# zerohd4869/MM-DFN

Measured on AMD Instinct MI355X. Metric: utterances/sec (fwd+bwd), IEMOCAP-shaped batch, higher is better.
Workload: dtype f32; 1 GPU; cfg2 (BASELINE configs[1]): B=16 dialogues/GPU, L=110, dims 100/100/512, 2 GCN layers, P=2, dropout 0.50; utterances_per_gpu=1760, parallelism=dp1

## Files before the change

mm_dfn_amd/csrc/gcn_stack.hip:

```cpp
#include "mmdfn_internal.h"
#include "../../include/mmdfn_hip.h"
#include "stack_image_map.h"
#include <stdlib.h>

namespace {

constexpr int RB = 16;

__device__ __forceinline__ float4 zero4() { return make_float4(0.f, 0.f, 0.f, 0.f); }
__device__ __forceinline__ float4 one4() { return make_float4(1.f, 1.f, 1.f, 1.f); }
__device__ __forceinline__ float4 mul4(float4 a, float4 b) { return make_float4(a.x * b.x, a.y * b.y, a.z * b.z, a.w * b.w); }
__device__ __forceinline__ float4 scl4(float4 a, float s) { return make_float4(a.x * s, a.y * s, a.z * s, a.w * s); }
__device__ __forceinline__ float4 add4(float4 a, float4 b) { return make_float4(a.x + b.x, a.y + b.y, a.z + b.z, a.w + b.w); }
__device__ __forceinline__ float4 fma4(float4 a, float s, float4 b) { return make_float4(a.x * s + b.x, a.y * s + b.y, a.z * s + b.z, a.w * s + b.w); }

typedef float f32x2_t __attribute__((ext_vector_type(2)));
__device__ __forceinline__ void st4_nt(float* p, float4 v) { __builtin_nontemporal_store((f32x4){v.x, v.y, v.z, v.w}, reinterpret_cast<f32x4*>(p)); }
__device__ __forceinline__ void nt_store2(float* p, float2 v) { __builtin_nontemporal_store((f32x2_t){v.x, v.y}, reinterpret_cast<f32x2_t*>(p)); }
__device__ __forceinline__ int frag_row(int i) { return i < 4 ? 2 * i : (i < 12 ? 2 * (i - 4) + 1 : 2 * (i - 12) + 8); }
__device__ __forceinline__ int frag_unit(int g) { return ((g & 1) << 1) | (g >> 1); }

__host__ __device__ inline int lds_stride(int K) {
    int ld = ((K + 15) & ~15) + 4;
    if (((ld >> 2) & 1) == 0) ld += 4;
// ... 904 lines not shown
        const float gi = rgi[s_].F, gf = rgf[s_].F, gg = rgg[s_].F, go = rgo[s_].F; \
        const float tc = tanhf_(rcn[s_].F);                                         \
        const float dhv = rdh[s_].F + rdh2[s_].F;                                   \
        const float dc = rdc[s_].F + dhv * go * (1.0f - tc * tc);                   \
        dO.F = dhv * tc * go * (1.0f - go);                                         \
        di.F = dc * gg * gi * (1.0f - gi);                                          \
        df.F = dc * rcp[s_].F * gf * (1.0f - gf);                                   \
        dg.F = dc * gi * (1.0f - gg * gg);                                          \
        dcp.F = dc * gf;                                                            \
    }
            GB1(x) GB1(y) GB1(z) GB1(w)
#undef GB1
            float* sp = dst + r * ldw + u;
            st4(sp, di); st4(sp + H, df); st4(sp + 2 * H, dg); st4(sp + 3 * H, dO);
            if (writer && row < R) {
                float* d = dG + (int64_t)row * 4 * H + u;
                st4(d, di); st4(d + H, df); st4(d + 2 * H, dg); st4(d + 3 * H, dO);
                if (has_h) st4(dc_prev + (int64_t)row * H + u, dcp);
            }
        }
    };
    if ((int)blockIdx.x < nrb) issue(blockIdx.x);
    wst.commit(sW, ldw, ncols, K);
    if (ncols < CBW) {
        for (int i = threadIdx.x; i < (CBW - ncols) * (ldw >> 2); i += 256) st4(sW + ncols * ldw + 4 * i, zero4());
    }
    zero_pads(sA, 2 * RB, ldw, K);
    if ((int)blockIdx.x < nrb) park(blockIdx.x, sA);
    __syncthreads();
    const int er = threadIdx.x >> 4, en = (threadIdx.x & 15) * 4;
    int buf = 0;
    FOR_ROW_BLOCKS(rb, nrb) {
        const int nxt = rb + gridDim.x;
        if (nxt < nrb) issue(nxt);
        const int erow = rb * RB + er;
        const bool eok = en < ncols && erow < R;
        const float4 rv = (!is_dh && dres && eok) ? ld4(dres + (int64_t)erow * lddres + n0 + en) : zero4();
        f32x4 acc[1] = {{0.f, 0.f, 0.f, 0.f}};
        float* Acur = sA + buf * RB * ldw;
        contract<1>(acc, wrow0, Acur, ldw, sW, ldw, K);
        __syncthreads();
        spill_tiles<1>(acc, wrow0, nt, Acur, ldp);
        __syncthreads();
        if (eok) {
            const float4 v = add4(ld4(Acur + er * ldp + en), rv);
            st4((is_dh ? dh_prev : dq) + (int64_t)erow * H + n0 + en, v);
        }
        if (nxt < nrb) park(nxt, sA + (buf ^ 1) * RB * ldw);
        __syncthreads();
        buf ^= 1;
    }
}

template <int ABL, bool WIDE = false, bool IMG = false>
__global__ __launch_bounds__(512) void lstm_gate_bwd_ws_kernel(const float* __restrict__ gates, const float* __restrict__ c_prev,
                                                               const float* __restrict__ c_new, const float* __restrict__ dh_a,
                                                               const float* __restrict__ dh_b, const float* __restrict__ dc_next,
                                                               const float* __restrict__ Wih, const float* __restrict__ Whh,
                                                               const float* __restrict__ dres, float* __restrict__ dG,
                                                               float* __restrict__ dc_prev, float* __restrict__ dq,
                                                               float* __restrict__ dh_prev, int R, int H, int has_h,
                                                               int lddres, const float4* __restrict__ img) {
    static_assert(!(IMG && WIDE), "the image form keeps the two-column-block launch");
    extern __shared__ __attribute__((aligned(16))) float smem[];
    const int K = 4 * H;
    const int ldw = lds_stride(K);
    float* sW = smem;
    float* sA = IMG ? smem : sW + CBW * ldw;
    const int nb = WIDE ? 1 : (H + CBW - 1) / CBW;
    const bool is_dh = (int)blockIdx.y >= nb;
    const int n0 = WIDE ? 0 : (is_dh ? blockIdx.y - nb : blockIdx.y) * CBW;
    const int ncols = min(CBW, H - n0);
    const int nrb = (R + RB - 1) / RB;
    const int tid = threadIdx.x & 255;
    const bool producer = threadIdx.x >= 256;
    const int nyb = gridDim.y, yb = blockIdx.y;
    const bool wr_i = (0 % nyb) == yb, wr_f = (1 % nyb) == yb, wr_g = (2 % nyb) == yb, wr_o = (3 % nyb) == yb, wr_c = yb == nyb - 1;
    const int H4 = H >> 2;
    const float rH4 = 1.0f / (float)H4;
    ImageFrags<1, IMG ? GATE_BWD_NKM : 1> wim;
    if constexpr (IMG) {
        const int cw = tid >> 6;
        const int tile0[1] = {16 * cw < ncols ? 16 * cw : 0};
        if (!producer) wim.load(img, tile0, CBW / 16, blockIdx.y, (K + 15) >> 4);
        const int np4 = (ldw - K) >> 2;
        const float rnp4 = 1.0f / (float)(np4 > 0 ? np4 : 1);
        for (int i = threadIdx.x; i < 2 * RB * np4; i += 512) { const int r = qdiv(i, rnp4), j = i - r * np4; st4(sA + r * ldw + K + 4 * j, zero4()); }
    } else {
        const float* Wsrc = is_dh ? Whh : Wih;
        const int inner = ncols >> 2;
        const int total = K * inner;
        constexpr int NW2 = 13;
        float4 v[NW2];
#pragma unroll
        for (int e = 0; e < NW2; ++e) {
            const int i0 = threadIdx.x + 512 * e, i = i0 < total ? i0 : total - 1;
            const int r = i / inner, j = i - r * inner;
            v[e] = ld4(Wsrc + (int64_t)r * H + n0 + 4 * j);
        }
#pragma unroll
        for (int e = 0; e < NW2; ++e) {
            const int i = threadIdx.x + 512 * e;
            if (i >= total) continue;
            const int r = i / inner, j = i - r * inner;
            float* d = sW + (4 * j) * ldw + r;
            d[0] = v[e].x; d[ldw] = v[e].y; d[2 * ldw] = v[e].z; d[3 * ldw] = v[e].w;
        }
        const int np4 = (ldw - K) >> 2;
        const float rnp4 = 1.0f / (float)(np4 > 0 ? np4 : 1);
        for (int i = threadIdx.x; i < ncols * np4; i += 512) { const int r = qdiv(i, rnp4), j = i - r * np4; st4(sW + r * ldw + K + 4 * j, zero4()); }
        for (int i = threadIdx.x; i < (CBW - ncols) * (ldw >> 2); i += 512) st4(sW + ncols * ldw + 4 * i, zero4());
        for (int i = threadIdx.x; i < 2 * RB * np4; i += 512) { const int r = qdiv(i, rnp4), j = i - r * np4; st4(sA + r * ldw + K + 4 * j, zero4()); }
    }
    constexpr int NS = 2;
    float4 rgi[NS], rgf[NS], rgg[NS], rgo[NS], rcn[NS], rcp[NS], rdh[NS], rdh2[NS], rdc[NS];
    auto issue = [&](int rb) {
#pragma unroll
        for (int s_ = 0; s_ < NS; ++s_) {
            const int i = tid + 256 * s_;
            const int r = qdiv(i, rH4), u = (i - r * H4) * 4, row = rb * RB + r;
            const bool ok = !(ABL & 2) && i < RB * H4 && row < R;
            const int64_t o = (int64_t)row * H + u;
            const float* gr = gates + (int64_t)row * 4 * H + u;
            rgi[s_] = ok ? ld4(gr) : zero4();
            rgf[s_] = ok ? ld4(gr + H) : zero4();
            rgg[s_] = ok ? ld4(gr + 2 * H) : zero4();
            rgo[s_] = ok ? ld4(gr + 3 * H) : zero4();
            rcn[s_] = ok ? ld4(c_new + o) : zero4();
            rcp[s_] = (ok && c_prev) ? ld4(c_prev + o) : zero4();
            rdh[s_] = (ok && dh_a) ? ld4(dh_a + o) : zero4();
            rdh2[s_] = (ok && dh_b) ? ld4(dh_b + o) : zero4();
            rdc[s_] = (ok && dc_next) ? ld4(dc_next + o) : zero4();
        }
    };
    float4 odi[NS], odf[NS], odg[NS], odo[NS], odc[NS];
    auto park = [&](float* dst) {
#pragma unroll
        for (int s_ = 0; s_ < NS; ++s_) {
            const int i = tid + 256 * s_;
            float4 di, df, dg, dO, dcp;
#define GB1(F)                                                                      \
    {                                                                               \
        const float gi = rgi[s_].F, gf = rgf[s_].F, gg = rgg[s_].F, go = rgo[s_].F; \
        const float tc = tanhf_(rcn[s_].F);                                         \
        const float dhv = rdh[s_].F + rdh2[s_].F;                                   \
        const float dc = rdc[s_].F + dhv * go * (1.0f - tc * tc);                   \
        dO.F = dhv * tc * go * (1.0f - go);                                         \
        di.F = dc * gg * gi * (1.0f - gi);                                          \
        df.F = dc * rcp[s_].F * gf * (1.0f - gf);                                   \
        dg.F = dc * gi * (1.0f - gg * gg);                                          \
        dcp.F = dc * gf;                                                            \
    }
            if (ABL & 4) { di = rgi[s_]; df = rgf[s_]; dg = rgg[s_]; dO = rgo[s_]; dcp = rcn[s_]; }
            else { GB1(x) GB1(y) GB1(z) GB1(w) }
#undef GB1
            odi[s_] = di; odf[s_] = df; odg[s_] = dg; odo[s_] = dO; odc[s_] = dcp;
            if (i >= RB * H4) continue;
            const int r = qdiv(i, rH4), u = (i - r * H4) * 4;
            float* sp = dst + r * ldw + u;
            st4(sp, di); st4(sp + H, df); st4(sp + 2 * H, dg); st4(sp + 3 * H, dO);
        }
    };
    auto flush = [&](int rb) {
        if (ABL & 8) return;
#pragma unroll
        for (int s_ = 0; s_ < NS; ++s_) {
            const int i = tid + 256 * s_;
            if (i >= RB * H4) continue;
            const int r = qdiv(i, rH4), u = (i - r * H4) * 4, row = rb * RB + r;
            if (row >= R) continue;
            float* d = dG + (int64_t)row * 4 * H + u;
            if (wr_i) st4_nt(d, odi[s_]);
            if (wr_f) st4_nt(d + H, odf[s_]);
            if (wr_g) st4_nt(d + 2 * H, odg[s_]);
            if (wr_o) st4_nt(d + 3 * H, odo[s_]);
            if (has_h && wr_c) st4(dc_prev + (int64_t)row * H + u, odc[s_]);
        }
    };
    const int first = blockIdx.x, stride = gridDim.x;
    if (producer) {
        if (first < nrb) { issue(first); park(sA); }
        if (first + stride < nrb) issue(first + stride);
        if (first < nrb) flush(first);
    }
    __syncthreads();
    const int w = tid >> 6, lane = tid & 63, fi = lane & 15, g = lane >> 4;
    const int wrow0[1] = {16 * w < ncols ? 16 * w : 0};
    const int ecol = n0 + 16 * w + frag_row(fi);
    const bool ecol_ok = (16 * w + frag_row(fi)) < ncols;
    float* const outp = is_dh ? dh_prev : dq;
    constexpr int NKC = WIDE ? GATE_BWD_WIDE_NKC : 1;
    const int ecol2 = CBW + 16 * w + frag_row(fi);
    const bool ecol2_ok = WIDE && ecol2 < H;
    const bool tile2 = WIDE && (CBW + 16 * w) < H;
    float4 wreg[NKC];
    if (WIDE && !producer) {
        const float* Wsrc = is_dh ? Whh : Wih;
        const int cc = ecol2_ok ? ecol2 : 0;
#pragma unroll
        for (int kc = 0; kc < NKC; ++kc) {
            const int k0 = 16 * kc + 4 * frag_unit(g);
            float v[4];
#pragma unroll
            for (int j = 0; j < 4; ++j) v[j] = (ecol2_ok && k0 + j < K) ? Wsrc[(int64_t)(k0 + j) * H + cc] : 0.f;
            wreg[kc] = make_float4(v[0], v[1], v[2], v[3]);
        }
    }
    int buf = 0;
    if (producer) {
        for (int rb = first; rb < nrb; rb += stride) {
            const int nxt = rb + stride;
            if (nxt < nrb) {
                park(sA + (buf ^ 1) * RB * ldw);
                if (nxt + stride < nrb) issue(nxt + stride);
                flush(nxt);
            }
            __syncthreads();
            buf ^= 1;
        }
        return;
    }
    for (int rb = first; rb < nrb; rb += stride) {
        {
            float rv[4];
#pragma unroll
            for (int r = 0; r < 4; ++r) {
                const int erow = rb * RB + frag_row(4 * g + r);
                rv[r] = (!is_dh && dres && ecol_ok && erow < R) ? dres[(int64_t)erow * lddres + ecol] : 0.f;
            }
            f32x4 acc[1] = {{0.f, 0.f, 0.f, 0.f}};
            if constexpr (WIDE) {
                float rv2[4];
#pragma unroll
                for (int r = 0; r < 4; ++r) {
                    const int erow = rb * RB + frag_row(4 * g + r);
                    rv2[r] = (!is_dh && dres && ecol2_ok && erow < R) ? dres[(int64_t)erow * lddres + ecol2] : 0.f;
                }
                f32x4 acc2 = {0.f, 0.f, 0.f, 0.f};
                const float* ap = sA + buf * RB * ldw + frag_row(fi) * ldw + 4 * frag_unit(g);
                const float* bp = sW + (wrow0[0] + frag_row(fi)) * ldw + 4 * frag_unit(g);
                const int nk = (K + 15) >> 4;
                float4 a_n = ld4(ap), b_n = ld4(bp);
#pragma unroll
                for (int kc = 0; kc < NKC; ++kc) {
                    if (kc < nk) {
                        const float4 a_c = a_n, b_c = b_n;
                        if (kc + 1 < nk) { a_n = ld4(ap + 16 * (kc + 1)); b_n = ld4(bp + 16 * (kc + 1)); }
                        const float av[4] = {a_c.x, a_c.y, a_c.z, a_c.w}, bv[4] = {b_c.x, b_c.y, b_c.z, b_c.w};
                        const float cv[4] = {wreg[kc].x, wreg[kc].y, wreg[kc].z, wreg[kc].w};
#pragma unroll
                        for (int j = 0; j < 4; ++j) {
                            acc[0] = __builtin_amdgcn_mfma_f32_16x16x4f32(av[j], bv[j], acc[0], 0, 0, 0);
                            if (tile2) acc2 = __builtin_amdgcn_mfma_f32_16x16x4f32(av[j], cv[j], acc2, 0, 0, 0);
                        }
                    }
                }
                if (ecol2_ok && !(ABL & 8)) {
#pragma unroll
                    for (int r = 0; r < 4; ++r) {
                        const int erow = rb * RB + frag_row(4 * g + r);
                        if (erow < R) outp[(int64_t)erow * H + ecol2] = acc2[r] + rv2[r];
                    }
                }
            } else {
                if constexpr (IMG) contract_img(acc, wim, sA + buf * RB * ldw, ldw, K);
                else if (!(ABL & 1)) contract<1>(acc, wrow0, sA + buf * RB * ldw, ldw, sW, ldw, K);
                else acc[0][0] = sA[buf * RB * ldw + fi * ldw + g];
            }
            if (ecol_ok && !(ABL & 8)) {
#pragma unroll
                for (int r = 0; r < 4; ++r) {
                    const int erow = rb * RB + frag_row(4 * g + r);
                    if (erow < R) outp[(int64_t)erow * H + ecol] = acc[0][r] + rv[r];
                }
            }
        }
        __syncthreads();
        buf ^= 1;
    }
}

template <bool IMG>
__global__ __launch_bounds__(512) void lstm_gate_fwd_ws_kernel(const float* __restrict__ q, const float* __restrict__ h,
                                                               const float* __restrict__ c, const float* __restrict__ Wih,
                                                               const float* __restrict__ Whh, const float* __restrict__ bsum, const float* __restrict__ bsum2,
                                                               float* __restrict__ gates, float* __restrict__ h_out,
                                                               float* __restrict__ c_out, int R, int H, int ldh,
                                                               const float4* __restrict__ img) {
    extern __shared__ __attribute__((aligned(16))) float smem[];
    const int K = h ? 2 * H : H;
    const int ldw = lds_stride(K), lde = UB + 4;
    float* sW = smem;
    float* sA = IMG ? smem : sW + 4 * UB * ldw;
    float* sE = sA + 2 * RB * ldw;
    const int u0 = blockIdx.y * UB;
    const int nu = min(UB, H - u0);
    const int H4 = H >> 2;
    const float rH4 = 1.0f / (float)H4;
    const int tid = threadIdx.x & 255;
    const bool producer = threadIdx.x >= 256;
    const int w = tid >> 6;
    const int wrow0[2] = {w * UB, w * UB + 16};
    ImageFrags<2, IMG ? GATE_FWD_NKM : 1> wim;
    if constexpr (IMG) {
        if (!producer) wim.load(img, wrow0, 4 * UB / 16, blockIdx.y, (K + 15) >> 4);
        const int np4 = (ldw - K) >> 2;
        const float rnp4 = 1.0f / (float)(np4 > 0 ? np4 : 1);
        for (int i = threadIdx.x; i < 2 * RB * np4; i += 512) { const int r = qdiv(i, rnp4), j = i - r * np4; st4(sA + r * ldw + K + 4 * j, zero4()); }
    }
    if constexpr (!IMG) {
        const int total = 4 * UB * H4;
        constexpr int NW2 = 7;
        float4 vi[NW2], vh[NW2];
#pragma unroll
        for (int e = 0; e < NW2; ++e) {
            const int i0 = threadIdx.x + 512 * e, i = i0 < total ? i0 : total - 1;
            const int rowl = qdiv(i, rH4), k = (i - rowl * H4) * 4;
            const int gate = rowl / UB, ul = rowl - gate * UB;
            const int64_t src = (int64_t)(gate * H + u0 + (ul < nu ? ul : nu - 1)) * H + k;
            vi[e] = ld4(Wih + src);
            vh[e] = h ? ld4(Whh + src) : zero4();
        }
#pragma unroll
        for (int e = 0; e < NW2; ++e) {
            const int i = threadIdx.x + 512 * e;
            if (i >= total) continue;
            const int rowl = qdiv(i, rH4), k = (i - rowl * H4) * 4;
            const int ul = rowl - (rowl / UB) * UB;
            st4(sW + rowl * ldw + k, ul < nu ? vi[e] : zero4());
            if (h) st4(sW + rowl * ldw + H + k, ul < nu ? vh[e] : zero4());
        }
        const int np4 = (ldw - K) >> 2;
        const float rnp4 = 1.0f / (float)(np4 > 0 ? np4 : 1);
        for (int i = threadIdx.x; i < 4 * UB * np4; i += 512) { const int r = qdiv(i, rnp4), j = i - r * np4; st4(sW + r * ldw + K + 4 * j, zero4()); }
        for (int i = threadIdx.x; i < 2 * RB * np4; i += 512) { const int r = qdiv(i, rnp4), j = i - r * np4; st4(sA + r * ldw + K + 4 * j, zero4()); }
    }
    const int nrb = (R + RB - 1) / RB;
    constexpr int NS = 2;
    float4 rq[NS], rh[NS];
    auto issue = [&](int rb) {
#pragma unroll
        for (int s = 0; s < NS; ++s) {
            const int i = tid + 256 * s;
            const int r = qdiv(i, rH4), k = (i - r * H4) * 4, row = rb * RB + r;
            const bool ok = i < RB * H4 && row < R;
            rq[s] = ok ? ld4(q + (int64_t)row * H + k) : zero4();
            rh[s] = (ok && h) ? ld4(h + (int64_t)row * ldh + k) : zero4();
        }
    };
    auto park = [&](float* dst) {
#pragma unroll
        for (int s = 0; s < NS; ++s) {
            const int i = tid + 256 * s;
            if (i >= RB * H4) continue;
            const int r = qdiv(i, rH4), k = (i - r * H4) * 4;
            st4(dst + r * ldw + k, rq[s]);
            if (h) st4(dst + r * ldw + H + k, rh[s]);
        }
    };
    const int er = tid >> 4, eu = (tid & 15) * 2;
    const bool ethread = eu < nu;
    float2 bi = make_float2(0.f, 0.f), bf = bi, bg = bi, bo = bi;
    if (producer && ethread) {
        bi = *reinterpret_cast<const float2*>(bsum + u0 + eu); bf = *reinterpret_cast<const float2*>(bsum + H + u0 + eu);
        bg = *reinterpret_cast<const float2*>(bsum + 2 * H + u0 + eu); bo = *reinterpret_cast<const float2*>(bsum + 3 * H + u0 + eu);
        if (bsum2) {
            const float2 ci = *reinterpret_cast<const float2*>(bsum2 + u0 + eu), cf = *reinterpret_cast<const float2*>(bsum2 + H + u0 + eu);
            const float2 cg = *reinterpret_cast<const float2*>(bsum2 + 2 * H + u0 + eu), co = *reinterpret_cast<const float2*>(bsum2 + 3 * H + u0 + eu);
            bi.x += ci.x; bi.y += ci.y; bf.x += cf.x; bf.y += cf.y; bg.x += cg.x; bg.y += cg.y; bo.x += co.x; bo.y += co.y;
        }
    }
    auto cell = [&](int rb, const float* E, float2 cp) {
        const int erow = rb * RB + er;
        if (!(ethread && erow < R)) return;
        const float2 pi = *reinterpret_cast<const float2*>(E + (0 * RB + er) * lde + eu);
        const float2 pf = *reinterpret_cast<const float2*>(E + (1 * RB + er) * lde + eu);
        const float2 pg = *reinterpret_cast<const float2*>(E + (2 * RB + er) * lde + eu);
        const float2 po = *reinterpret_cast<const float2*>(E + (3 * RB + er) * lde + eu);
        float2 gi, gf, gg, go, cn, hn;
#define K8F(F_)                                                                 \
    {                                                                           \
        gi.F_ = sigmoidf_(pi.F_ + bi.F_); gf.F_ = sigmoidf_(pf.F_ + bf.F_); gg.F_ = tanhf_(pg.F_ + bg.F_); go.F_ = sigmoidf_(po.F_ + bo.F_); \
        cn.F_ = gf.F_ * cp.F_ + gi.F_ * gg.F_;                                  \
        hn.F_ = go.F_ * tanhf_(cn.F_);                                          \
    }
        K8F(x) K8F(y)
#undef K8F
        float* gr = gates + (int64_t)erow * 4 * H + u0 + eu;
        nt_store2(gr, gi); nt_store2(gr + H, gf); nt_store2(gr + 2 * H, gg); nt_store2(gr + 3 * H, go);
        *reinterpret_cast<float2*>(c_out + (int64_t)erow * H + u0 + eu) = cn;
        *reinterpret_cast<float2*>(h_out + (int64_t)erow * ldh + u0 + eu) = hn;
    };
    auto load_c = [&](int rb) {
        const int erow = rb * RB + er;
        return (c && ethread && erow < R) ? *reinterpret_cast<const float2*>(c + (int64_t)erow * H + u0 + eu) : make_float2(0.f, 0.f);
    };
    const int first = blockIdx.x, stride = gridDim.x;
    float2 cp_prev = make_float2(0.f, 0.f);
    if (producer) {
        if (first < nrb) { issue(first); park(sA); cp_prev = load_c(first); }
        if (first + stride < nrb) issue(first + stride);
    }
    __syncthreads();
    int buf = 0, prev_rb = -1;
    for (int rb = first; rb < nrb; rb += stride) {
        const int nxt = rb + stride;
        if (producer) {
            if (prev_rb >= 0) cell(prev_rb, sE + (buf ^ 1) * 4 * RB * lde, cp_prev);
            cp_prev = load_c(rb);
            if (nxt < nrb) {
                park(sA + (buf ^ 1) * RB * ldw);
                if (nxt + stride < nrb) issue(nxt + stride);
            }
        } else {
            f32x4 acc[2] = {{0.f, 0.f, 0.f, 0.f}, {0.f, 0.f, 0.f, 0.f}};
            if constexpr (IMG) contract_img(acc, wim, sA + buf * RB * ldw, ldw, K);
            else contract<2>(acc, wrow0, sA + buf * RB * ldw, ldw, sW, ldw, K);
            const int lane = tid & 63, fi = lane & 15, g = lane >> 4;
            float* E = sE + buf * 4 * RB * lde;
#pragma unroll
            for (int t = 0; t < 2; ++t)
#pragma unroll
                for (int r = 0; r < 4; ++r) E[(w * RB + frag_row(4 * g + r)) * lde + 16 * t + frag_row(fi)] = acc[t][r];
        }
        __syncthreads();
        prev_rb = rb;
        buf ^= 1;
    }
    if (producer && prev_rb >= 0) cell(prev_rb, sE + (buf ^ 1) * 4 * RB * lde, cp_prev);
}

inline bool bad_dims(int64_t R, int H) { return R <= 0 || H < 4 || (H & 3) || H > 100 || R > (int64_t)1 << 30; }

inline bool gate_ws(int R) {
#ifdef MMDFN_TUNING
    if (const char* e = getenv("MMDFN_GATE_WS")) return atoi(e) != 0;
#endif
    return R >= 64;
}

constexpr int LAYER_WS_ROWS = 64;
inline bool layer_ws(int R) {
#ifdef MMDFN_TUNING
    if (const char* e = getenv("MMDFN_LAYER_WS")) return atoi(e) != 0;
#endif
    return R >= LAYER_WS_ROWS;
}

constexpr int GATE_SPLIT_ROWS = 16384;
constexpr int GATE_BWD_WIDE_ROWS = 16384;
inline bool gate_split(int R, int H) {
#ifdef MMDFN_TUNING
    if (const char* e = getenv("MMDFN_GATE_SPLIT")) return atoi(e) != 0;
#endif
    return R >= GATE_SPLIT_ROWS && H >= 32;
}

inline int row_groups(int R, int column_blocks) {
    const int nrb = (R + RB - 1) / RB;
    int gq = (256 + column_blocks - 1) / column_blocks;
    if (gq > nrb) gq = nrb;
    const int per = (nrb + gq - 1) / gq;
    gq = (nrb + per - 1) / per;
    return gq < 1 ? 1 : gq;
}

#define LAUNCH_BIG_LDS(kern, grid, lds, stream, ...)                                  \
    do {                                                                              \
        if ((lds) > 156 * 1024) return -1;                                            \
        if (int e_ = mmdfn_allow_big_lds(kern)) return e_;                            \
        hipLaunchKernelGGL(kern, grid, dim3(256), lds, (hipStream_t)(stream), __VA_ARGS__); \
        MMDFN_CHECK_LAUNCH();                                                         \
    } while (0)

}

extern "C" int mmdfn_gcn_input_fwd(const float* x, const float* mx, const float* W0, const float* b0, const float* m0,
                                   float* xd, float* h0, float* cur0, int R, int F, int H, int ldxd, float mscale,
                                   void* stream) {
    if (bad_dims(R, H) || F < 4 || (F & 3) || F > 256 || ldxd < F || (ldxd & 3)) return -1;
    const size_t lds = ((size_t)(H + 2 * RB) * lds_stride(F) + RB * (((H + 15) & ~15) + 4)) * sizeof(float);
    LAUNCH_BIG_LDS(gcn_input_fwd_kernel<false>, dim3(row_groups(R, 1)), lds, stream, x, mx, W0, b0, m0, xd, h0, cur0, R, F, H, ldxd,
                   mscale, (const float4*)nullptr);
    return 0;
}

extern "C" int mmdfn_gcn_input_bwd(const float* dcur0, const float* m0, const float* dh0, const float* h0, const float* W0,
                                   const float* dxd, const float* mx, float* dpre, float* dx, int R, int F, int H, int lddxd,
                                   float mscale, void* stream) {
    if (bad_dims(R, H) || F < 4 || (F & 3) || F > 256 || (dxd && (lddxd < F || (lddxd & 3)))) return -1;
    const size_t lds = ((size_t)(F + 2 * RB) * lds_stride(H) + RB * (((F + 15) & ~15) + 4)) * sizeof(float);
    LAUNCH_BIG_LDS(gcn_input_bwd_kernel<false>, dim3(row_groups(R, 1)), lds, stream, dcur0, m0, dh0, h0, W0, dxd, mx, dpre, dx, R, F, H,
                   lddxd, mscale, (const float4*)nullptr);
    return 0;
}

static int lstm_gate_fwd_impl(const float* q, const float* h, const float* c, const float* Wih, const float* Whh,
                              const float* bsum, const float* bsum2, float* gates, float* h_out, float* c_out, int R, int H,
                              int ldh, const void* planes, void* stream);

extern "C" int mmdfn_lstm_gate_fwd_ld(const float* q, const float* h, const float* c, const float* Wih, const float* Whh,
                                      const float* bsum, const float* bsum2, float* gates, float* h_out, float* c_out, int R, int H,
                                      int ldh, void* stream) {
    return lstm_gate_fwd_impl(q, h, c, Wih, Whh, bsum, bsum2, gates, h_out, c_out, R, H, ldh, nullptr, stream);
}

extern "C" int64_t mmdfn_lstm_gate_planes_workspace(int H) { return (H < 8 || (H & 3)) ? -1 : mmdfn_lstm_gate_planes_floats(H); }
extern "C" int mmdfn_lstm_gate_cut_weights(const float* Wih, const float* Whh, float* planes, int H, void* stream) {
    return mmdfn_launch_lstm_gate_cut(Wih, Whh, planes, H, (hipStream_t)stream);
}
extern "C" int mmdfn_lstm_gate_fwd_pre(const float* q, const float* h, const float* c, const float* Wih, const float* Whh,
                                       const float* bsum, const float* bsum2, float* gates, float* h_out, float* c_out, int R,
                                       int H, int ldh, const float* planes, void* stream) {
    return lstm_gate_fwd_impl(q, h, c, Wih, Whh, bsum, bsum2, gates, h_out, c_out, R, H, ldh, planes, stream);
}
extern "C" int mmdfn_lstm_gate_takes_planes(int R, int H) { return (!bad_dims(R, H) && gate_split(R, H)) ? 1 : 0; }

static int lstm_gate_fwd_impl(const float* q, const float* h, const float* c, const float* Wih, const float* Whh,
                              const float* bsum, const float* bsum2, float* gates, float* h_out, float* c_out, int R, int H,
                              int ldh, const void* planes, void* stream) {
    if (bad_dims(R, H) || (h == nullptr) != (c == nullptr) || ldh < H || (ldh & 3)) return -1;
    if (gate_split(R, H)) {
        const int rc = mmdfn_launch_lstm_gate_fwd_split(q, h, c, Wih, Whh, bsum, bsum2, gates, h_out, c_out, R, H,
                                                        ldh, planes, (hipStream_t)stream);
        if (rc != -2) return rc;
    }
    const int ncb = (H + UB - 1) / UB;
    if (gate_ws(R)) {
        const size_t ldsw = ((size_t)(4 * UB + 2 * RB) * lds_stride(h ? 2 * H : H) + 2 * 4 * RB * (UB + 4)) * sizeof(float);
        if (ldsw > 156 * 1024) return -1;
        if (int e_ = mmdfn_allow_big_lds(lstm_gate_fwd_ws_kernel<false>)) return e_;
        hipLaunchKernelGGL(lstm_gate_fwd_ws_kernel<false>, dim3(row_groups(R, ncb), ncb), dim3(512), ldsw, (hipStream_t)stream, q, h, c, Wih,
                           Whh, bsum, bsum2, gates, h_out, c_out, R, H, ldh, (const float4*)nullptr);
        MMDFN_CHECK_LAUNCH();
        return 0;
    }
    const size_t lds = ((size_t)(4 * UB + 2 * RB) * lds_stride(h ? 2 * H : H) + 4 * RB * (UB + 4)) * sizeof(float);
    LAUNCH_BIG_LDS(lstm_gate_fwd_kernel, dim3(row_groups(R, ncb), ncb), lds, stream, q, h, c, Wih, Whh, bsum, bsum2, gates,
                   h_out, c_out, R, H, ldh);
    return 0;
}

extern "C" int mmdfn_lstm_gate_fwd(const float* q, const float* h, const float* c, const float* Wih, const float* Whh,
                                   const float* bsum, const float* bsum2, float* gates, float* h_out, float* c_out, int R, int H,
                                   void* stream) {
    return mmdfn_lstm_gate_fwd_ld(q, h, c, Wih, Whh, bsum, bsum2, gates, h_out, c_out, R, H, H, stream);
}

extern "C" int mmdfn_lstm_gate_bwd(const float* gates, const float* c_prev, const float* c_new, const float* dh_a,
                                   const float* dh_b, const float* dc_next, const float* Wih, const float* Whh,
                                   const float* dres, float* dG, float* dc_prev, float* dq, float* dh_prev, int R, int H,
                                   int has_h, int lddres, void* stream) {
    if (bad_dims(R, H) || (has_h && (dc_prev == nullptr || dh_prev == nullptr || c_prev == nullptr))) return -1;
    if (dres != nullptr && (lddres < H || (lddres & 3))) return -1;
    const int nb = (H + CBW - 1) / CBW;
    const int ncb = has_h ? 2 * nb : nb;
    if (gate_ws(R)) {
        const size_t ldsw = (size_t)(CBW + 2 * RB) * lds_stride(4 * H) * sizeof(float);
        if (ldsw > 156 * 1024) return -1;
#ifdef MMDFN_TUNING
#define GBWS_ABL(A_)                                                                                                         \
    case A_:                                                                                                                 \
        if (int e_ = mmdfn_allow_big_lds(lstm_gate_bwd_ws_kernel<A_>)) return e_;                                            \
        hipLaunchKernelGGL(lstm_gate_bwd_ws_kernel<A_>, dim3(row_groups(R, ncb), ncb), dim3(512), ldsw, (hipStream_t)stream, \
                           gates, c_prev, c_new, dh_a, dh_b, dc_next, Wih, Whh, dres, dG, dc_prev, dq, dh_prev, R, H, has_h, \
                           lddres, (const float4*)nullptr);                                                                                      \
        MMDFN_CHECK_LAUNCH();                                                                                                \
        return 0;
        if (const char* e = getenv("MMDFN_GATE_ABL")) {
            switch (atoi(e)) {
                GBWS_ABL(1) GBWS_ABL(2) GBWS_ABL(4) GBWS_ABL(8) GBWS_ABL(3) GBWS_ABL(6) GBWS_ABL(7) GBWS_ABL(15) GBWS_ABL(12) GBWS_ABL(14)
                default: break;
            }
        }
#undef GBWS_ABL
#endif
        bool wide = H > CBW && 4 * H <= 16 * GATE_BWD_WIDE_NKC && R >= GATE_BWD_WIDE_ROWS;
#ifdef MMDFN_TUNING
        if (const char* e = getenv("MMDFN_GATE_BWD_WIDE")) wide = H > CBW && 4 * H <= 16 * GATE_BWD_WIDE_NKC && atoi(e) != 0;
#endif
        if (wide) {
            const int ncw = has_h ? 2 : 1;
            if (int e_ = mmdfn_allow_big_lds(lstm_gate_bwd_ws_kernel<0, true>)) return e_;
            hipLaunchKernelGGL((lstm_gate_bwd_ws_kernel<0, true>), dim3(row_groups(R, ncw), ncw), dim3(512), ldsw, (hipStream_t)stream,
                               gates, c_prev, c_new, dh_a, dh_b, dc_next, Wih, Whh, dres, dG, dc_prev, dq, dh_prev, R, H, has_h, lddres,
                               (const float4*)nullptr);
            MMDFN_CHECK_LAUNCH();
            return 0;
        }
        if (int e_ = mmdfn_allow_big_lds(lstm_gate_bwd_ws_kernel<0>)) return e_;
        hipLaunchKernelGGL(lstm_gate_bwd_ws_kernel<0>, dim3(row_groups(R, ncb), ncb), dim3(512), ldsw, (hipStream_t)stream, gates,
                           c_prev, c_new, dh_a, dh_b, dc_next, Wih, Whh, dres, dG, dc_prev, dq, dh_prev, R, H, has_h, lddres,
                           (const float4*)nullptr);
        MMDFN_CHECK_LAUNCH();
        return 0;
    }
    const size_t lds = (size_t)(CBW + 2 * RB) * lds_stride(4 * H) * sizeof(float);
    LAUNCH_BIG_LDS(lstm_gate_bwd_kernel, dim3(row_groups(R, ncb), ncb), lds, stream, gates, c_prev, c_new, dh_a, dh_b, dc_next,
                   Wih, Whh, dres, dG, dc_prev, dq, dh_prev, R, H, has_h, lddres);
    return 0;
}

extern "C" int mmdfn_gcnii_layer_fwd(const float* hi, const float* h0, const float* W, const float* q, const float* m,
                                     float* out, float* gmask, float theta, float alpha, int R, int H, int ldo, float mscale,
                                     void* stream) {
    if (bad_dims(R, H) || ldo < H || (ldo & 3)) return -1;
    if (layer_ws(R)) {
        const size_t ldsw = ((size_t)(H + 2 * RB) * lds_stride(2 * H) + 2 * RB * (((H + 15) & ~15) + 4)) * sizeof(float);
        if (ldsw > 156 * 1024) return -1;
        if (int e_ = mmdfn_allow_big_lds(gcnii_layer_fwd_ws_kernel)) return e_;
        hipLaunchKernelGGL(gcnii_layer_fwd_ws_kernel, dim3(row_groups(R, 1)), dim3(512), ldsw, (hipStream_t)stream, hi, h0, W, q, m,
                           out, gmask, theta, alpha, R, H, ldo, mscale);
        MMDFN_CHECK_LAUNCH();
        return 0;
    }
    const size_t lds = ((size_t)(H + 2 * RB) * lds_stride(2 * H) + RB * (((H + 15) & ~15) + 4)) * sizeof(float);
    LAUNCH_BIG_LDS(gcnii_layer_fwd_kernel, dim3(row_groups(R, 1)), lds, stream, hi, h0, W, q, m, out, gmask, theta, alpha, R, H,
                   ldo, mscale);
    return 0;
}

extern "C" int mmdfn_gcnii_layer_bwd_ld(const float* dout, const float* gmask, const float* W, float* dP, float* dhi, float* dh0,
                                        float theta, float alpha, int R, int H, int lddo, int acc_h0, int lddhi, void* stream) {
    if (bad_dims(R, H) || lddo < H || (lddo & 3) || lddhi < H || (lddhi & 3) || !(theta > 0.f)) return -1;
    if (layer_ws(R)) {
        const size_t ldsw = ((size_t)(2 * H + 2 * RB) * lds_stride(H) + 2 * RB * (((2 * H + 15) & ~15) + 4)) * sizeof(float);
        if (ldsw > 156 * 1024) return -1;
        if (int e_ = mmdfn_allow_big_lds(gcnii_layer_bwd_ws_kernel<false>)) return e_;
        hipLaunchKernelGGL(gcnii_layer_bwd_ws_kernel<false>, dim3(row_groups(R, 1)), dim3(512), ldsw, (hipStream_t)stream, dout, gmask, W,
                           dP, dhi, dh0, theta, alpha, R, H, lddo, acc_h0, lddhi, (const float4*)nullptr);
        MMDFN_CHECK_LAUNCH();
        return 0;
    }
    const size_t lds = ((size_t)(2 * H + 2 * RB) * lds_stride(H) + RB * (((2 * H + 15) & ~15) + 4)) * sizeof(float);
    LAUNCH_BIG_LDS(gcnii_layer_bwd_kernel, dim3(row_groups(R, 1)), lds, stream, dout, gmask, W, dP, dhi, dh0, theta, alpha, R, H,
                   lddo, acc_h0, lddhi);
    return 0;
}

extern "C" int mmdfn_gcnii_layer_bwd(const float* dout, const float* gmask, const float* W, float* dP, float* dhi, float* dh0,
                                     float theta, float alpha, int R, int H, int lddo, int acc_h0, void* stream) {
    return mmdfn_gcnii_layer_bwd_ld(dout, gmask, W, dP, dhi, dh0, theta, alpha, R, H, lddo, acc_h0, H, stream);
}

namespace {

constexpr int INPUT_FWD_IMG_BLOCKS = 1, INPUT_BWD_IMG_BLOCKS = 1, LAYER_BWD_IMG_BLOCKS = 2;
inline int img_row_groups(int R, int per) {
// ... 99 lines not shown
```

Baseline: 2.407 million utterances/s.

## Add register prefetch ring to LSTM gate warp-specialized kernels with unconditional clamped loads

```diff
diff --git a/mm_dfn_amd/csrc/gcn_stack.hip b/mm_dfn_amd/csrc/gcn_stack.hip
--- a/mm_dfn_amd/csrc/gcn_stack.hip
+++ b/mm_dfn_amd/csrc/gcn_stack.hip
@@ -980,7 +980,8 @@
     }
 }
 
-template <int ABL, bool WIDE = false, bool IMG = false>
+constexpr int GATE_RING_D = 1;
+template <int ABL, bool WIDE = false, bool IMG = false, int D = GATE_RING_D>
 __global__ __launch_bounds__(512) void lstm_gate_bwd_ws_kernel(const float* __restrict__ gates, const float* __restrict__ c_prev,
                                                                const float* __restrict__ c_new, const float* __restrict__ dh_a,
                                                                const float* __restrict__ dh_b, const float* __restrict__ dc_next,
@@ -1001,20 +1002,59 @@
     const int ncols = min(CBW, H - n0);
     const int nrb = (R + RB - 1) / RB;
     const int tid = threadIdx.x & 255;
-    const bool producer = threadIdx.x >= 256;
+    const bool producer = __builtin_amdgcn_readfirstlane((int)threadIdx.x) >= 256;
     const int nyb = gridDim.y, yb = blockIdx.y;
     const bool wr_i = (0 % nyb) == yb, wr_f = (1 % nyb) == yb, wr_g = (2 % nyb) == yb, wr_o = (3 % nyb) == yb, wr_c = yb == nyb - 1;
     const int H4 = H >> 2;
     const float rH4 = 1.0f / (float)H4;
+    const int first = blockIdx.x, stride = gridDim.x;
+    const int last = first < nrb ? first + ((nrb - 1 - first) / stride) * stride : 0;
+    constexpr int NS = 2;
+    float4 rgi[D][NS], rgf[D][NS], rgg[D][NS], rgo[D][NS], rcn[D][NS], rcp[D][NS], rdh[D][NS], rdh2[D][NS], rdc[D][NS];
+    const float* const cpP = c_prev ? c_prev : c_new;
+    const float* const dhaP = dh_a ? dh_a : c_new;
+    const float* const dhbP = dh_b ? dh_b : c_new;
+    const float* const dcnP = dc_next ? dc_next : c_new;
+    auto issue = [&](const int sl, int rb) {
+        if (rb > last) rb = last;
+#pragma unroll
+        for (int s_ = 0; s_ < NS; ++s_) {
+            if (ABL & 2) {
+                rgi[sl][s_] = rgf[sl][s_] = rgg[sl][s_] = rgo[sl][s_] = rcn[sl][s_] = rcp[sl][s_] = rdh[sl][s_] = rdh2[sl][s_] = rdc[sl][s_] = zero4();
+                continue;
+            }
+            const int i = min(tid + 256 * s_, RB * H4 - 1);
+            const int r = qdiv(i, rH4), u = (i - r * H4) * 4, row = min(rb * RB + r, R - 1);
+            const int64_t o = (int64_t)row * H + u;
+            const float* gr = gates + (int64_t)row * 4 * H + u;
+            rgi[sl][s_] = ld4(gr);
+            rgf[sl][s_] = ld4(gr + H);
+            rgg[sl][s_] = ld4(gr + 2 * H);
+            rgo[sl][s_] = ld4(gr + 3 * H);
+            rcn[sl][s_] = ld4(c_new + o);
+            rcp[sl][s_] = ld4(cpP + o);
+            rdh[sl][s_] = ld4(dhaP + o);
+            rdh2[sl][s_] = ld4(dhbP + o);
+            rdc[sl][s_] = ld4(dcnP + o);
+        }
+    };
+    auto issue_ring = [&]() {
+        if (producer && first < nrb) {
+#pragma unroll
+            for (int d = 0; d < D; ++d) issue(d, first + d * stride);
+        }
+    };
     ImageFrags<1, IMG ? GATE_BWD_NKM : 1> wim;
     if constexpr (IMG) {
         const int cw = tid >> 6;
         const int tile0[1] = {16 * cw < ncols ? 16 * cw : 0};
         if (!producer) wim.load(img, tile0, CBW / 16, blockIdx.y, (K + 15) >> 4);
+        issue_ring();
         const int np4 = (ldw - K) >> 2;
         const float rnp4 = 1.0f / (float)(np4 > 0 ? np4 : 1);
         for (int i = threadIdx.x; i < 2 * RB * np4; i += 512) { const int r = qdiv(i, rnp4), j = i - r * np4; st4(sA + r * ldw + K + 4 * j, zero4()); }
     } else {
+        issue_ring();
         const float* Wsrc = is_dh ? Whh : Wih;
         const int inner = ncols >> 2;
         const int total = K * inner;
@@ -1028,8 +1068,7 @@
         }
 #pragma unroll
         for (int e = 0; e < NW2; ++e) {
-            const int i = threadIdx.x + 512 * e;
-            if (i >= total) continue;
+            const int i0 = threadIdx.x + 512 * e, i = i0 < total ? i0 : total - 1;
             const int r = i / inner, j = i - r * inner;
             float* d = sW + (4 * j) * ldw + r;
             d[0] = v[e].x; d[ldw] = v[e].y; d[2 * ldw] = v[e].z; d[3 * ldw] = v[e].w;
@@ -1040,51 +1079,35 @@
         for (int i = threadIdx.x; i < (CBW - ncols) * (ldw >> 2); i += 512) st4(sW + ncols * ldw + 4 * i, zero4());
         for (int i = threadIdx.x; i < 2 * RB * np4; i += 512) { const int r = qdiv(i, rnp4), j = i - r * np4; st4(sA + r * ldw + K + 4 * j, zero4()); }
     }
-    constexpr int NS = 2;
-    float4 rgi[NS], rgf[NS], rgg[NS], rgo[NS], rcn[NS], rcp[NS], rdh[NS], rdh2[NS], rdc[NS];
-    auto issue = [&](int rb) {
+    float4 odi[NS], odf[NS], odg[NS], odo[NS], odc[NS];
+    auto park = [&](const int sl, int rb, float* dst) {
 #pragma unroll
         for (int s_ = 0; s_ < NS; ++s_) {
             const int i = tid + 256 * s_;
-            const int r = qdiv(i, rH4), u = (i - r * H4) * 4, row = rb * RB + r;
-            const bool ok = !(ABL & 2) && i < RB * H4 && row < R;
-            const int64_t o = (int64_t)row * H + u;
-            const float* gr = gates + (int64_t)row * 4 * H + u;
-            rgi[s_] = ok ? ld4(gr) : zero4();
-            rgf[s_] = ok ? ld4(gr + H) : zero4();
-            rgg[s_] = ok ? ld4(gr + 2 * H) : zero4();
-            rgo[s_] = ok ? ld4(gr + 3 * H) : zero4();
-            rcn[s_] = ok ? ld4(c_new + o) : zero4();
-            rcp[s_] = (ok && c_prev) ? ld4(c_prev + o) : zero4();
-            rdh[s_] = (ok && dh_a) ? ld4(dh_a + o) : zero4();
-            rdh2[s_] = (ok && dh_b) ? ld4(dh_b + o) : zero4();
-            rdc[s_] = (ok && dc_next) ? ld4(dc_next + o) : zero4();
-        }
-    };
-    float4 odi[NS], odf[NS], odg[NS], odo[NS], odc[NS];
-    auto park = [&](float* dst) {
-#pragma unroll
-        for (int s_ = 0; s_ < NS; ++s_) {
-            const int i = tid + 256 * s_;
+            const int r = qdiv(min(i, RB * H4 - 1), rH4), u = (min(i, RB * H4 - 1) - r * H4) * 4;
+            const bool ok = i < RB * H4 && rb * RB + r < R;
+            const float4 vgi = ok ? rgi[sl][s_] : zero4(), vgf = ok ? rgf[sl][s_] : zero4(), vgg = ok ? rgg[sl][s_] : zero4();
+            const float4 vgo = ok ? rgo[sl][s_] : zero4(), vcn = ok ? rcn[sl][s_] : zero4();
+            const float4 vcp = (ok && c_prev) ? rcp[sl][s_] : zero4(), vdh = (ok && dh_a) ? rdh[sl][s_] : zero4();
+            const float4 vdh2 = (ok && dh_b) ? rdh2[sl][s_] : zero4(), vdc = (ok && dc_next) ? rdc[sl][s_] : zero4();
             float4 di, df, dg, dO, dcp;
 #define GB1(F)                                                                      \
     {                                                                               \
-        const float gi = rgi[s_].F, gf = rgf[s_].F, gg = rgg[s_].F, go = rgo[s_].F; \
-        const float tc = tanhf_(rcn[s_].F);                                         \
-        const float dhv = rdh[s_].F + rdh2[s_].F;                                   \
-        const float dc = rdc[s_].F + dhv * go * (1.0f - tc * tc);                   \
+        const float gi = vgi.F, gf = vgf.F, gg = vgg.F, go = vgo.F;                 \
+        const float tc = tanhf_(vcn.F);                                             \
+        const float dhv = vdh.F + vdh2.F;                                           \
+        const float dc = vdc.F + dhv * go * (1.0f - tc * tc);                       \
         dO.F = dhv * tc * go * (1.0f - go);                                         \
         di.F = dc * gg * gi * (1.0f - gi);                                          \
-        df.F = dc * rcp[s_].F * gf * (1.0f - gf);                                   \
+        df.F = dc * vcp.F * gf * (1.0f - gf);                                       \
         dg.F = dc * gi * (1.0f - gg * gg);                                          \
         dcp.F = dc * gf;                                                            \
     }
-            if (ABL & 4) { di = rgi[s_]; df = rgf[s_]; dg = rgg[s_]; dO = rgo[s_]; dcp = rcn[s_]; }
+            if (ABL & 4) { di = vgi; df = vgf; dg = vgg; dO = vgo; dcp = vcn; }
             else { GB1(x) GB1(y) GB1(z) GB1(w) }
 #undef GB1
             odi[s_] = di; odf[s_] = df; odg[s_] = dg; odo[s_] = dO; odc[s_] = dcp;
             if (i >= RB * H4) continue;
-            const int r = qdiv(i, rH4), u = (i - r * H4) * 4;
             float* sp = dst + r * ldw + u;
             st4(sp, di); st4(sp + H, df); st4(sp + 2 * H, dg); st4(sp + 3 * H, dO);
         }
@@ -1105,11 +1128,10 @@
             if (has_h && wr_c) st4(dc_prev + (int64_t)row * H + u, odc[s_]);
         }
     };
-    const int first = blockIdx.x, stride = gridDim.x;
-    if (producer) {
-        if (first < nrb) { issue(first); park(sA); }
-        if (first + stride < nrb) issue(first + stride);
-        if (first < nrb) flush(first);
+    if (producer && first < nrb) {
+        park(0, first, sA);
+        issue(0, first + D * stride);
+        flush(first);
     }
     __syncthreads();
     const int w = tid >> 6, lane = tid & 63, fi = lane & 15, g = lane >> 4;
@@ -1117,6 +1139,7 @@
     const int ecol = n0 + 16 * w + frag_row(fi);
     const bool ecol_ok = (16 * w + frag_row(fi)) < ncols;
     float* const outp = is_dh ? dh_prev : dq;
+    const bool use_res = !is_dh && dres != nullptr;
     constexpr int NKC = WIDE ? GATE_BWD_WIDE_NKC : 1;
     const int ecol2 = CBW + 16 * w + frag_row(fi);
     const bool ecol2_ok = WIDE && ecol2 < H;
@@ -1134,35 +1157,70 @@
             wreg[kc] = make_float4(v[0], v[1], v[2], v[3]);
         }
     }
+    auto store_tile = [&](const f32x4& a, const float (&res)[4], int col, bool col_ok, int rb) {
+        if (ABL & 8) return;
+        float o[4];
+#pragma unroll
+        for (int r = 0; r < 4; ++r) {
+            o[r] = a[r] + res[r];
+            asm volatile("" : "+v"(o[r]));
+        }
+#pragma unroll
+        for (int r = 0; r < 4; ++r) {
+            const int erow = rb * RB + frag_row(4 * g + r);
+            if (col_ok && erow < R) outp[(int64_t)erow * H + col] = o[r];
+        }
+    };
     int buf = 0;
     if (producer) {
-        for (int rb = first; rb < nrb; rb += stride) {
-            const int nxt = rb + stride;
-            if (nxt < nrb) {
-                park(sA + (buf ^ 1) * RB * ldw);
-                if (nxt + stride < nrb) issue(nxt + stride);
+        if (first >= nrb) return;
+        const int n_it = (last - first) / stride;
+        int rb = first;
+        for (int round = n_it / D; round > 0; --round) {
+#pragma unroll
+            for (int s = 0; s < D; ++s) {
+                const int nxt = rb + stride;
+                park((s + 1) % D, nxt, sA + (buf ^ 1) * RB * ldw);
+                issue((s + 1) % D, nxt + D * stride);
                 flush(nxt);
+                __syncthreads();
+                buf ^= 1;
+                rb = nxt;
             }
-            __syncthreads();
-            buf ^= 1;
-        }
+        }
+#pragma unroll
+        for (int s = 0; s + 1 < D; ++s) {
+            if (s < n_it % D) {
+                const int nxt = rb + stride;
+                park((s + 1) % D, nxt, sA + (buf ^ 1) * RB * ldw);
+                flush(nxt);
+                __syncthreads();
+                buf ^= 1;
+                rb = nxt;
+            }
+        }
+        __syncthreads();
         return;
     }
     for (int rb = first; rb < nrb; rb += stride) {
         {
-            float rv[4];
-#pragma unroll
-            for (int r = 0; r < 4; ++r) {
-                const int erow = rb * RB + frag_row(4 * g + r);
-                rv[r] = (!is_dh && dres && ecol_ok && erow < R) ? dres[(int64_t)erow * lddres + ecol] : 0.f;
+            float rv[4] = {0.f, 0.f, 0.f, 0.f};
+            if (use_res) {
+#pragma unroll
+                for (int r = 0; r < 4; ++r) {
+                    const int erow = min(rb * RB + frag_row(4 * g + r), R - 1);
+                    rv[r] = dres[(int64_t)erow * lddres + (ecol_ok ? ecol : n0)];
+                }
             }
             f32x4 acc[1] = {{0.f, 0.f, 0.f, 0.f}};
             if constexpr (WIDE) {
-                float rv2[4];
-#pragma unroll
-                for (int r = 0; r < 4; ++r) {
-                    const int erow = rb * RB + frag_row(4 * g + r);
-                    rv2[r] = (!is_dh && dres && ecol2_ok && erow < R) ? dres[(int64_t)erow * lddres + ecol2] : 0.f;
+                float rv2[4] = {0.f, 0.f, 0.f, 0.f};
+                if (use_res) {
+#pragma unroll
+                    for (int r = 0; r < 4; ++r) {
+                        const int erow = min(rb * RB + frag_row(4 * g + r), R - 1);
+                        rv2[r] = dres[(int64_t)erow * lddres + (ecol2_ok ? ecol2 : 0)];
+                    }
                 }
                 f32x4 acc2 = {0.f, 0.f, 0.f, 0.f};
                 const float* ap = sA + buf * RB * ldw + frag_row(fi) * ldw + 4 * frag_unit(g);
@@ -1183,32 +1241,21 @@
                         }
                     }
                 }
-                if (ecol2_ok && !(ABL & 8)) {
-#pragma unroll
-                    for (int r = 0; r < 4; ++r) {
-                        const int erow = rb * RB + frag_row(4 * g + r);
-                        if (erow < R) outp[(int64_t)erow * H + ecol2] = acc2[r] + rv2[r];
-                    }
-                }
+                store_tile(acc2, rv2, ecol2, ecol2_ok, rb);
             } else {
                 if constexpr (IMG) contract_img(acc, wim, sA + buf * RB * ldw, ldw, K);
                 else if (!(ABL & 1)) contract<1>(acc, wrow0, sA + buf * RB * ldw, ldw, sW, ldw, K);
                 else acc[0][0] = sA[buf * RB * ldw + fi * ldw + g];
             }
-            if (ecol_ok && !(ABL & 8)) {
-#pragma unroll
-                for (int r = 0; r < 4; ++r) {
-                    const int erow = rb * RB + frag_row(4 * g + r);
-                    if (erow < R) outp[(int64_t)erow * H + ecol] = acc[0][r] + rv[r];
-                }
-            }
+            store_tile(acc[0], rv, ecol, ecol_ok, rb);
         }
         __syncthreads();
         buf ^= 1;
     }
 }
 
-template <bool IMG>
+constexpr int GATE_FWD_RING_D = 1;
+template <bool IMG, int D = GATE_FWD_RING_D, bool NT = true>
 __global__ __launch_bounds__(512) void lstm_gate_fwd_ws_kernel(const float* __restrict__ q, const float* __restrict__ h,
                                                                const float* __restrict__ c, const float* __restrict__ Wih,
                                                                const float* __restrict__ Whh, const float* __restrict__ bsum, const float* __restrict__ bsum2,
@@ -1226,17 +1273,42 @@
     const int H4 = H >> 2;
     const float rH4 = 1.0f / (float)H4;
     const int tid = threadIdx.x & 255;
-    const bool producer = threadIdx.x >= 256;
+    const bool producer = __builtin_amdgcn_readfirstlane((int)threadIdx.x) >= 256;
     const int w = tid >> 6;
     const int wrow0[2] = {w * UB, w * UB + 16};
+    const int nrb = (R + RB - 1) / RB;
+    const int first = blockIdx.x, stride = gridDim.x;
+    const int last = first < nrb ? first + ((nrb - 1 - first) / stride) * stride : 0;
+    constexpr int NS = 2;
+    float4 rq[D][NS], rh[D][NS];
+    const float* const hP = h ? h : q;
+    const int ldhP = h ? ldh : H;
+    auto issue = [&](const int sl, int rb) {
+        if (rb > last) rb = last;
+#pragma unroll
+        for (int s = 0; s < NS; ++s) {
+            const int i = min(tid + 256 * s, RB * H4 - 1);
+            const int r = qdiv(i, rH4), k = (i - r * H4) * 4, row = min(rb * RB + r, R - 1);
+            rq[sl][s] = ld4(q + (int64_t)row * H + k);
+            rh[sl][s] = ld4(hP + (int64_t)row * ldhP + k);
+        }
+    };
+    auto issue_ring = [&]() {
+        if (producer && first < nrb) {
+#pragma unroll
+            for (int d = 0; d < D; ++d) issue(d, first + d * stride);
+        }
+    };
     ImageFrags<2, IMG ? GATE_FWD_NKM : 1> wim;
     if constexpr (IMG) {
         if (!producer) wim.load(img, wrow0, 4 * UB / 16, blockIdx.y, (K + 15) >> 4);
+        issue_ring();
         const int np4 = (ldw - K) >> 2;
         const float rnp4 = 1.0f / (float)(np4 > 0 ? np4 : 1);
         for (int i = threadIdx.x; i < 2 * RB * np4; i += 512) { const int r = qdiv(i, rnp4), j = i - r * np4; st4(sA + r * ldw + K + 4 * j, zero4()); }
     }
     if constexpr (!IMG) {
+        issue_ring();
         const int total = 4 * UB * H4;
         constexpr int NW2 = 7;
         float4 vi[NW2], vh[NW2];
@@ -1251,8 +1323,7 @@
         }
 #pragma unroll
         for (int e = 0; e < NW2; ++e) {
-            const int i = threadIdx.x + 512 * e;
-            if (i >= total) continue;
+            const int i0 = threadIdx.x + 512 * e, i = i0 < total ? i0 : total - 1;
             const int rowl = qdiv(i, rH4), k = (i - rowl * H4) * 4;
             const int ul = rowl - (rowl / UB) * UB;
             st4(sW + rowl * ldw + k, ul < nu ? vi[e] : zero4());
@@ -1263,27 +1334,16 @@
         for (int i = threadIdx.x; i < 4 * UB * np4; i += 512) { const int r = qdiv(i, rnp4), j = i - r * np4; st4(sW + r * ldw + K + 4 * j, zero4()); }
         for (int i = threadIdx.x; i < 2 * RB * np4; i += 512) { const int r = qdiv(i, rnp4), j = i - r * np4; st4(sA + r * ldw + K + 4 * j, zero4()); }
     }
-    const int nrb = (R + RB - 1) / RB;
-    constexpr int NS = 2;
-    float4 rq[NS], rh[NS];
-    auto issue = [&](int rb) {
+    auto park = [&](const int sl, int rb, float* dst) {
 #pragma unroll
         for (int s = 0; s < NS; ++s) {
             const int i = tid + 256 * s;
-            const int r = qdiv(i, rH4), k = (i - r * H4) * 4, row = rb * RB + r;
-            const bool ok = i < RB * H4 && row < R;
-            rq[s] = ok ? ld4(q + (int64_t)row * H + k) : zero4();
-            rh[s] = (ok && h) ? ld4(h + (int64_t)row * ldh + k) : zero4();
-        }
-    };
-    auto park = [&](float* dst) {
-#pragma unroll
-        for (int s = 0; s < NS; ++s) {
-            const int i = tid + 256 * s;
+            const int r = qdiv(min(i, RB * H4 - 1), rH4), k = (min(i, RB * H4 - 1) - r * H4) * 4;
+            const bool ok = rb * RB + r < R;
+            const float4 vq = ok ? rq[sl][s] : zero4(), vh = ok ? rh[sl][s] : zero4();
             if (i >= RB * H4) continue;
-            const int r = qdiv(i, rH4), k = (i - r * H4) * 4;
-            st4(dst + r * ldw + k, rq[s]);
-            if (h) st4(dst + r * ldw + H + k, rh[s]);
+            st4(dst + r * ldw + k, vq);
+            if (h) st4(dst + r * ldw + H + k, vh);
         }
     };
     const int er = tid >> 4, eu = (tid & 15) * 2;
@@ -1315,7 +1375,12 @@
         K8F(x) K8F(y)
 #undef K8F
         float* gr = gates + (int64_t)erow * 4 * H + u0 + eu;
-        nt_store2(gr, gi); nt_store2(gr + H, gf); nt_store2(gr + 2 * H, gg); nt_store2(gr + 3 * H, go);
+        if constexpr (NT) {
+            nt_store2(gr, gi); nt_store2(gr + H, gf); nt_store2(gr + 2 * H, gg); nt_store2(gr + 3 * H, go);
+        } else {
+            *reinterpret_cast<float2*>(gr) = gi; *reinterpret_cast<float2*>(gr + H) = gf;
+            *reinterpret_cast<float2*>(gr + 2 * H) = gg; *reinterpret_cast<float2*>(gr + 3 * H) = go;
+        }
         *reinterpret_cast<float2*>(c_out + (int64_t)erow * H + u0 + eu) = cn;
         *reinterpret_cast<float2*>(h_out + (int64_t)erow * ldh + u0 + eu) = hn;
     };
@@ -1323,39 +1388,56 @@
         const int erow = rb * RB + er;
         return (c && ethread && erow < R) ? *reinterpret_cast<const float2*>(c + (int64_t)erow * H + u0 + eu) : make_float2(0.f, 0.f);
     };
-    const int first = blockIdx.x, stride = gridDim.x;
     float2 cp_prev = make_float2(0.f, 0.f);
+    if (producer && first < nrb) {
+        park(0, first, sA);
+        issue(0, first + D * stride);
+        cp_prev = load_c(first);
+    }
+    __syncthreads();
+    int buf = 0;
     if (producer) {
-        if (first < nrb) { issue(first); park(sA); cp_prev = load_c(first); }
-        if (first + stride < nrb) issue(first + stride);
-    }
-    __syncthreads();
-    int buf = 0, prev_rb = -1;
+        if (first >= nrb) return;
+        int rb = first, prev_rb = -1;
+        auto block = [&](const int sl, const bool req) {
+            const int nxt = rb + stride;
+            park(sl, nxt, sA + (buf ^ 1) * RB * ldw);
+            if (req) issue(sl, nxt + D * stride);
+            const float2 cp = load_c(rb);
+            if (prev_rb >= 0) cell(prev_rb, sE + (buf ^ 1) * 4 * RB * lde, cp_prev);
+            cp_prev = cp;
+            __syncthreads();
+            prev_rb = rb;
+            rb = nxt;
+            buf ^= 1;
+        };
+        const int n_it = (last - first) / stride;
+        for (int round = n_it / D; round > 0; --round) {
+#pragma unroll
+            for (int s = 0; s < D; ++s) block((s + 1) % D, true);
+        }
+#pragma unroll
+        for (int s = 0; s + 1 < D; ++s)
+            if (s < n_it % D) block((s + 1) % D, false);
+        const float2 cp = load_c(rb);
+        if (prev_rb >= 0) cell(prev_rb, sE + (buf ^ 1) * 4 * RB * lde, cp_prev);
+        __syncthreads();
+        cell(rb, sE + buf * 4 * RB * lde, cp);
+        return;
+    }
     for (int rb = first; rb < nrb; rb += stride) {
-        const int nxt = rb + stride;
-        if (producer) {
-            if (prev_rb >= 0) cell(prev_rb, sE + (buf ^ 1) * 4 * RB * lde, cp_prev);
-            cp_prev = load_c(rb);
-            if (nxt < nrb) {
-                park(sA + (buf ^ 1) * RB * ldw);
-                if (nxt + stride < nrb) issue(nxt + stride);
-            }
-        } else {
-            f32x4 acc[2] = {{0.f, 0.f, 0.f, 0.f}, {0.f, 0.f, 0.f, 0.f}};
-            if constexpr (IMG) contract_img(acc, wim, sA + buf * RB * ldw, ldw, K);
-            else contract<2>(acc, wrow0, sA + buf * RB * ldw, ldw, sW, ldw, K);
-            const int lane = tid & 63, fi = lane & 15, g = lane >> 4;
-            float* E = sE + buf * 4 * RB * lde;
-#pragma unroll
-            for (int t = 0; t < 2; ++t)
-#pragma unroll
-                for (int r = 0; r < 4; ++r) E[(w * RB + frag_row(4 * g + r)) * lde + 16 * t + frag_row(fi)] = acc[t][r];
-        }
-        __syncthreads();
-        prev_rb = rb;
+        f32x4 acc[2] = {{0.f, 0.f, 0.f, 0.f}, {0.f, 0.f, 0.f, 0.f}};
+        if constexpr (IMG) contract_img(acc, wim, sA + buf * RB * ldw, ldw, K);
+        else contract<2>(acc, wrow0, sA + buf * RB * ldw, ldw, sW, ldw, K);
+        const int lane = tid & 63, fi = lane & 15, g = lane >> 4;
+        float* E = sE + buf * 4 * RB * lde;
+#pragma unroll
+        for (int t = 0; t < 2; ++t)
+#pragma unroll
+            for (int r = 0; r < 4; ++r) E[(w * RB + frag_row(4 * g + r)) * lde + 16 * t + frag_row(fi)] = acc[t][r];
+        __syncthreads();
         buf ^= 1;
     }
-    if (producer && prev_rb >= 0) cell(prev_rb, sE + (buf ^ 1) * 4 * RB * lde, cp_prev);
 }
 
 inline bool bad_dims(int64_t R, int H) { return R <= 0 || H < 4 || (H & 3) || H > 100 || R > (int64_t)1 << 30; }
@@ -1457,11 +1539,27 @@
     if (gate_ws(R)) {
         const size_t ldsw = ((size_t)(4 * UB + 2 * RB) * lds_stride(h ? 2 * H : H) + 2 * 4 * RB * (UB + 4)) * sizeof(float);
         if (ldsw > 156 * 1024) return -1;
-        if (int e_ = mmdfn_allow_big_lds(lstm_gate_fwd_ws_kernel<false>)) return e_;
-        hipLaunchKernelGGL(lstm_gate_fwd_ws_kernel<false>, dim3(row_groups(R, ncb), ncb), dim3(512), ldsw, (hipStream_t)stream, q, h, c, Wih,
-                           Whh, bsum, bsum2, gates, h_out, c_out, R, H, ldh, (const float4*)nullptr);
-        MMDFN_CHECK_LAUNCH();
-        return 0;
+#define GFWS_LAUNCH(D_, NT_)                                                                                                \
+    do {                                                                                                                    \
+        if (int e_ = mmdfn_allow_big_lds(lstm_gate_fwd_ws_kernel<false, D_, NT_>)) return e_;                              \
+        hipLaunchKernelGGL((lstm_gate_fwd_ws_kernel<false, D_, NT_>), dim3(row_groups(R, ncb), ncb), dim3(512), ldsw,      \
+                           (hipStream_t)stream, q, h, c, Wih, Whh, bsum, bsum2, gates, h_out, c_out, R, H, ldh,           \
+                           (const float4*)nullptr);                                                                        \
+        MMDFN_CHECK_LAUNCH();                                                                                               \
+        return 0;                                                                                                           \
+    } while (0)
+#ifdef MMDFN_TUNING
+        {
+            const char *ed = getenv("MMDFN_GATE_FWD_RING"), *en = getenv("MMDFN_GATE_FWD_NT");
+            const int d = ed ? atoi(ed) : GATE_FWD_RING_D;
+            const bool nt = en ? atoi(en) != 0 : true;
+            if (d == 2 && nt) GFWS_LAUNCH(2, true);
+            if (d == 2) GFWS_LAUNCH(2, false);
+            if (!nt) GFWS_LAUNCH(1, false);
+        }
+#endif
+        GFWS_LAUNCH(GATE_FWD_RING_D, true);
+#undef GFWS_LAUNCH
     }
     const size_t lds = ((size_t)(4 * UB + 2 * RB) * lds_stride(h ? 2 * H : H) + 4 * RB * (UB + 4)) * sizeof(float);
     LAUNCH_BIG_LDS(lstm_gate_fwd_kernel, dim3(row_groups(R, ncb), ncb), lds, stream, q, h, c, Wih, Whh, bsum, bsum2, gates,
@@ -1507,21 +1605,27 @@
 #ifdef MMDFN_TUNING
         if (const char* e = getenv("MMDFN_GATE_BWD_WIDE")) wide = H > CBW && 4 * H <= 16 * GATE_BWD_WIDE_NKC && atoi(e) != 0;
 #endif
-        if (wide) {
-            const int ncw = has_h ? 2 : 1;
-            if (int e_ = mmdfn_allow_big_lds(lstm_gate_bwd_ws_kernel<0, true>)) return e_;
-            hipLaunchKernelGGL((lstm_gate_bwd_ws_kernel<0, true>), dim3(row_groups(R, ncw), ncw), dim3(512), ldsw, (hipStream_t)stream,
-                               gates, c_prev, c_new, dh_a, dh_b, dc_next, Wih, Whh, dres, dG, dc_prev, dq, dh_prev, R, H, has_h, lddres,
-                               (const float4*)nullptr);
-            MMDFN_CHECK_LAUNCH();
-            return 0;
-        }
-        if (int e_ = mmdfn_allow_big_lds(lstm_gate_bwd_ws_kernel<0>)) return e_;
-        hipLaunchKernelGGL(lstm_gate_bwd_ws_kernel<0>, dim3(row_groups(R, ncb), ncb), dim3(512), ldsw, (hipStream_t)stream, gates,
-                           c_prev, c_new, dh_a, dh_b, dc_next, Wih, Whh, dres, dG, dc_prev, dq, dh_prev, R, H, has_h, lddres,
-                           (const float4*)nullptr);
-        MMDFN_CHECK_LAUNCH();
-        return 0;
+        const int ncw = wide ? (has_h ? 2 : 1) : ncb;
+#define GBWS_LAUNCH(W_, D_)                                                                                                  \
+    do {                                                                                                                     \
+        if (int e_ = mmdfn_allow_big_lds(lstm_gate_bwd_ws_kernel<0, W_, false, D_>)) return e_;                             \
+        hipLaunchKernelGGL((lstm_gate_bwd_ws_kernel<0, W_, false, D_>), dim3(row_groups(R, ncw), ncw), dim3(512), ldsw,     \
+                           (hipStream_t)stream, gates, c_prev, c_new, dh_a, dh_b, dc_next, Wih, Whh, dres, dG, dc_prev, dq, \
+                           dh_prev, R, H, has_h, lddres, (const float4*)nullptr);                                           \
+        MMDFN_CHECK_LAUNCH();                                                                                                \
+        return 0;                                                                                                            \
+    } while (0)
+#ifdef MMDFN_TUNING
+        if (const char* e = getenv("MMDFN_GATE_RING")) {
+            const int d = atoi(e);
+            if (d == 2 && wide) GBWS_LAUNCH(true, 2);
+            if (d == 2) GBWS_LAUNCH(false, 2);
+            if (d == 3 && !wide) GBWS_LAUNCH(false, 3);
+        }
+#endif
+        if (wide) GBWS_LAUNCH(true, GATE_RING_D);
+        GBWS_LAUNCH(false, GATE_RING_D);
+#undef GBWS_LAUNCH
     }
     const size_t lds = (size_t)(CBW + 2 * RB) * lds_stride(4 * H) * sizeof(float);
     LAUNCH_BIG_LDS(lstm_gate_bwd_kernel, dim3(row_groups(R, ncb), ncb), lds, stream, gates, c_prev, c_new, dh_a, dh_b, dc_next,
```

Result: no change. 2.407 million utterances/s, median of 2 (-0.0%).
